# 21cmfast/21cmFAST

Hardware: AMD Instinct MI355X
Metric: IonizeBox cells/sec (512^3 HII_DIM, 40 filter radii) (higher is better)
Workload: dtype f32; 1 GPU; ComputeIonizedBox single-z, HII_DIM=512, 40 filter steps, G=2 (delta tophat + n_ion exp-MFP), first snapshot, device-resident inputs; hii_dim=512, n_radii=40, filtered_grids=2, parallelism=single GPU, fft=native

## Files before the change

### 21cmfast_amd/csrc/hip/c21hip.h

```cpp
#ifndef C21HIP_H
#define C21HIP_H

#include <stddef.h>

#include "ws_slots.h"

#ifdef __cplusplus
extern "C" {
#endif

int c21hip_device_count(void);
int c21hip_current_device(void);
int c21hip_use_device(int device);
int c21hip_is_device_ptr(const void *p);
void *c21hip_ws(int slot, size_t bytes);
__attribute__((visibility("hidden"))) const void *c21_stage_in(int slot, const void *p, size_t bytes, void *stream, int *status);
void *c21hip_ws_peek(int slot, size_t *bytes);
int c21hip_ws_adopt(int slot, void *ptr, size_t bytes);
void *c21hip_raw_alloc(size_t bytes);
void *c21hip_vmm_chunk(size_t phys_bytes, size_t map_bytes, void **va_out);
void c21hip_vmm_chunk_free(void *chunk);
int c21hip_ws_adopt_vmm(int slot, void *chunk, size_t bytes);
void c21hip_raw_free(void *p);
size_t c21hip_free_bytes(void);
// ... 37 lines not shown
                           void *stream);
int c21hip_split_filter_c2r(const float *split_src, float *split_work, float *real_out,
                            long out_zstride, int nx, int ny, int nz, double box_len,
                            double box_len_z, int filter_type, float R, float R_param, int apply,
                            void *stream);

int c21hip_split_r2c(const float *real_in, long in_zstride, float *split_out, int nx, int ny,
                     int nz, double factor, double lo, double hi, float out_scale, void *stream);
int c21hip_split_filter_xy(const float *split_src, float *split_work, int nx, int ny, int nz,
                           double box_len, double box_len_z, int filter_type, float R,
                           float R_param, int apply, void *stream);
int c21hip_split_filter_xy2(const float *src_a, float *work_a, int filter_a, float R_param_a,
                            const float *src_b, float *work_b, int filter_b, float R_param_b,
                            int nx, int ny, int nz, double box_len, double box_len_z, float R,
                            int apply, int table_slot, int tables_ready, void *stream);
int c21hip_split_filter_shell(const float *src_a, float *work_a, int filter_a, const float *src_b,
                              float *work_b, int filter_b, int n_grids, int nx, int ny, int nz,
                              double box_len, double box_len_z, float R_inner, float R_outer,
                              float R_star, int apply, void *stream);
int c21hip_split_filter_xy2_pair(const float *src_a, float *work_a, float *work_a2, int filter_a,
                                 float R_param_a, const float *src_b, float *work_b,
                                 float *work_b2, int filter_b, float R_param_b, int nx, int ny,
                                 int nz, double box_len, double box_len_z, float R, float R2,
                                 int table_slot, int table_slot2, int phases, void *stream);
int c21hip_split_filter_x_pair1(const float *src, float *work, float *work2, int filter_type, int nx, int ny,
                                int nz, double box_len, double box_len_z, float R, float R2, int phases,
                                void *stream);
int c21hip_split_filter_xy2_pair_eval(const float *src_a, float *work_a, float *work_a2, int filter_a,
                                      const float *src_b, float *work_b, float *work_b2, int filter_b, int nx,
                                      int ny, int nz, double box_len, double box_len_z, float R, float R2,
// ... 591 lines not shown
```

### 21cmfast_amd/csrc/hip/fft_native.hip

```cpp
#include <hip/hip_runtime.h>

#include <cmath>
#include <map>
#include <mutex>
#include <vector>

#include "c21hip.h"
#include "fcoll_device.h"
#include "ms_window.h"
#include "c21cm_abi.h"
#include "c21cm_grid.h"

#ifndef C21X_XPAIR_THREADS
#define C21X_XPAIR_THREADS 512
#endif
#ifndef C21X_FUSE512
#define C21X_FUSE512 1
#endif
#ifndef C21X_FUSE1024
#define C21X_FUSE1024 1
#endif
#ifndef C21X_F512_MERGE
#define C21X_F512_MERGE 1
#endif
// ... 505 lines not shown
    long line_stride, line_bstride, outer_stride, outer_bstride, col_stride;
    int line_lb, outer_lb;
    int n_outer, filter_axis;
    int og, ct, npair;
    const wtab_t *wt0, *wt1;
};

template <int N, int SIGN, int FMODE>
__global__ void __launch_bounds__((LineThreads<N, FMODE>::value), (LineThreads<N, FMODE>::value / 256))
line_pass_kernel(LinePassArgs a, const float2 *__restrict__ tw_global) {
    static_assert(N >= 64, "tile loader needs N >= 64");
    constexpr int kBlock = LineThreads<N, FMODE>::value;
    constexpr int TZ = line_tile_cols(N);
    constexpr int CPAIR = TZ / 2;
    constexpr int RSTEP = kBlock / CPAIR;
    constexpr bool WEVAL = (FMODE >= 6 && FMODE <= 9);
    constexpr bool WDIRECT = (FMODE == 8 || FMODE == 9);
    constexpr bool WIN = (FMODE == 3 || (FMODE == 5 && !C21X_XPAIR_NOWIN) || WEVAL);
    constexpr bool PAIR = (FMODE == 5 || FMODE == 7 || FMODE == 9);
    constexpr int NR = PAIR ? 2 : 1;
    using LineItem = LineItemT<PAIR>;
    extern __shared__ float4 lds_raw[];
    float2 *tile = reinterpret_cast<float2 *>(lds_raw);
    float2 *tw = tile + NR * N * TZ;
    float2 *tw_half = tw + N;
    float *wnodes = reinterpret_cast<float *>(tw_half + (N >= 1024 ? N / 2 : 0));
    for (int t = threadIdx.x; t < N; t += kBlock) tw[t] = tw_global[t];
    if (N >= 1024)
        for (int t = threadIdx.x; t < N / 2; t += kBlock) tw_half[t] = tw_global[2 * t];
    if constexpr (WEVAL) {
        const int per = 3 * a.wev_n_nodes;
        for (int t = threadIdx.x; t < per; t += kBlock) {
// ... 98 lines not shown
        const int outer = mi == 0 ? it.og : it.n_outer - it.og;
        return (long)(outer >> it.outer_lb) * it.outer_bstride +
               (long)(outer & ((1 << it.outer_lb) - 1)) * it.outer_stride +
               (long)it.ct * TZ * it.col_stride;
    };
    auto row_off = [](const LineItem &it, int r) {
        return (unsigned)(r >> it.line_lb) * (unsigned)it.line_bstride +
               (unsigned)(r & ((1 << it.line_lb) - 1)) * (unsigned)it.line_stride;
    };

    constexpr bool TWO_SETS = (N < 1024) && (!PAIR || C21X_XPAIR_TWO_SETS);
    float4 reg_a[2 * NP], reg_b[2 * NP];
    constexpr bool F512 = C21X_FUSE512 && N == 512 && kBlock == 512 && (FMODE == 0 || WEVAL);
    constexpr bool F1024 = C21X_FUSE1024 && N == 1024 && kBlock == 512 && (FMODE == 0 || FMODE == 3 || WEVAL);
    constexpr bool FUSED = F512 || F1024;
    constexpr int NW = FUSED ? 2 * NP : NP;
    constexpr bool WPRE = (N >= 512) && !FUSED;
    float2 wpre[NR][WPRE ? NP : 1], wcur[NR][NW], wpre_half[NR], wcur_half[NR];
    auto w_reload = [&](const LineItem &it, int m) {
        const int mi = it.npair == 2 ? (m & 1) : 0;
        return m == 0 || (a.dual && mi == 0);
    };
    struct KAbs {
        float kh, kl;
    };
    auto k_abs = [](float kx, float ky, float kz) -> KAbs {
        const float ksq = __fadd_rn(__fadd_rn(__fmul_rn(kx, kx), __fmul_rn(ky, ky)), __fmul_rn(kz, kz));
        KAbs k;
        k.kh = __builtin_amdgcn_sqrtf(ksq);
        const float r = __fmaf_rn(-k.kh, k.kh, ksq);
// ... 215 lines not shown
    auto process = [&](float4(&reg)[2 * NP], const TileRef &cur, const TileRef &nxt,
                       const TileRef &refill) {
        const LineItem &it = cur.it;
        const int m = cur.m;
        const long st_half = (long)((N / 2) >> it.line_lb) * it.line_bstride;
        if (!first) __syncthreads();
        first = false;
        if (WIN && WPRE && w_reload(it, m)) {
#pragma unroll
            for (int rr = 0; rr < NR; rr++) {
#pragma unroll
                for (int u = 0; u < NP; u++) wcur[rr][u] = wpre[rr][WPRE ? u : 0];
                wcur_half[rr] = wpre_half[rr];
            }
        }
        double op_c0 = 1., op_c1 = 1.;
        if (FMODE == 4) {
            const int c0 = it.ct * TZ + 2 * c4;
            int kyi0, kyi1, kzi0, kzi1;
            if (it.filter_axis == 0) {
                const int mi = it.npair == 2 ? (m & 1) : 0;
                const int outer = mi == 0 ? it.og : it.n_outer - it.og;
                kyi0 = kyi1 = (outer <= a.n_y / 2) ? outer : outer - a.n_y;
                kzi0 = c0;
                kzi1 = c0 + 1;
            } else {
                kyi0 = (c0 <= a.n_y / 2) ? c0 : c0 - a.n_y;
                kyi1 = (c0 + 1 <= a.n_y / 2) ? c0 + 1 : c0 + 1 - a.n_y;
                kzi0 = kzi1 = a.n_z / 2;
            }
// ... 883 lines not shown
    hipStream_t stream;
    KTimeScope(int kind, hipStream_t s) : stream(s) {
        if (!g_ktime_on) return;
        if (hipEventCreate(&r.e0) != hipSuccess || hipEventCreate(&r.e1) != hipSuccess) return;
        r.kind = kind;
        (void)hipEventRecord(r.e0, stream);
    }
    ~KTimeScope() {
        if (r.kind < 0) return;
        (void)hipEventRecord(r.e1, stream);
        g_ktime.push_back(r);
    }
};
constexpr int ktime_kind(int sign, int fmode) {
    return sign < 0 ? 9 : (fmode == 0 ? 1 : fmode == 3 ? 0 : fmode == 5 ? 6 : (fmode == 6 || fmode == 8) ? 7
                                                              : (fmode == 7 || fmode == 9) ? 8 : 10);
}

static bool ynyq_split_on() {
    static int on = -1;
    if (on < 0) {
        const char *e = getenv("C21CM_YNYQ_SPLIT");
        on = (e && atoi(e) == 0) ? 0 : 1;
    }
    return on != 0;
}

#ifndef C21X_XORDER_DEFAULT
#define C21X_XORDER_DEFAULT 3
#endif
template <int N, int SIGN, int FMODE>
int launch_line_pass_mode(const LinePassArgs &a, hipStream_t stream) {
    const float2 *tw = twiddles(N);
    if (!tw) {
        c21hip_set_error("native FFT: twiddle table allocation failed");
        return C21CM_MEMORY_ALLOC_ERROR;
    }
    const size_t lds = sizeof(float2) * ((size_t)((FMODE == 5 || FMODE == 7 || FMODE == 9) ? 2 : 1) * N *
                                             line_tile_cols(N) + N + (N >= 1024 ? N / 2 : 0)) +
                       ((FMODE >= 6 && FMODE <= 9) ? sizeof(float) * 3 * (size_t)a.wev_n_nodes * a.wev_n_tabs : 0);
    if (lds > 160 * 1024) {
        c21hip_set_error("native FFT: %zu bytes of LDS for a %d-point line pass (mode %d)", lds, N, FMODE);
        return C21CM_VALUE_ERROR;
    }
    if (FMODE != 0 && a.n_geo > 1 && a.g1_strided) {
        c21hip_set_error("native FFT: a strided second geometry in a line pass of mode %d", FMODE);
        return C21CM_VALUE_ERROR;
    }
    const bool epi_split = ynyq_split_on() && a.n_geo > 1 && a.g1_strided && a.g1.line_bstride == 1 &&
                           a.g1.line_lb == 0 && a.g1.col_stride % 2 == 0;
    const int n_work = geo_items(a.g0) + (a.n_geo > 1 ? geo_items(a.g1) : 0);
    int per_cu = (int)((160 * 1024) / lds) > 0 ? (int)((160 * 1024) / lds) : 1;
    const int by_waves = (LineThreads<N, FMODE>::value >= 512 && N > 256) ? 1 : 2;
    if (per_cu > by_waves) per_cu = by_waves;
    int nblocks = 256 * per_cu;
// ... 23 lines not shown
}

template <int N, int SIGN>
int launch_line_pass(const LinePassArgs &a, int fmode, hipStream_t stream) {
    if (SIGN > 0 && fmode == 3) return launch_line_pass_mode<N, +1, 3>(a, stream);
    if (SIGN > 0 && fmode == 4) return launch_line_pass_mode<N, +1, 4>(a, stream);
    if constexpr (N <= 512)
        if (SIGN > 0 && fmode == 5) return launch_line_pass_mode<N, +1, 5>(a, stream);
    if constexpr (N >= 128 && (N & (N - 1)) == 0) {
        if (SIGN > 0 && fmode == 6) return launch_line_pass_mode<N, +1, 6>(a, stream);
        if (SIGN > 0 && fmode == 8) return launch_line_pass_mode<N, +1, 8>(a, stream);
        if constexpr (N <= 512) {
            if (SIGN > 0 && fmode == 7) return launch_line_pass_mode<N, +1, 7>(a, stream);
            if (SIGN > 0 && fmode == 9) return launch_line_pass_mode<N, +1, 9>(a, stream);
        }
    }
    if (fmode >= 6 && fmode <= 9) {
        c21hip_set_error("native FFT: evaluated windows are not built for %d-point lines", N);
        return C21CM_VALUE_ERROR;
    }
    return launch_line_pass_mode<N, SIGN, 0>(a, stream);
}

template <int SIGN>
int dispatch_line_pass(int n, const LinePassArgs &a, int fmode, hipStream_t stream) {
    switch (n) {
        case 64: return launch_line_pass<64, SIGN>(a, fmode, stream);
        case 128: return launch_line_pass<128, SIGN>(a, fmode, stream);
        case 192: return launch_line_pass<192, SIGN>(a, fmode, stream);
        case 256: return launch_line_pass<256, SIGN>(a, fmode, stream);
// ... 1828 lines not shown
    if (env && env[0] == 't') return 0;
    return wev_static_ok(filter_a, filter_b, n_grids, nx, ny, nz, 1, nullptr, nullptr) ? 1 : 0;
}
extern "C" int c21hip_split_filter_xy_single_pair(const float *src, float *work, float *work2,
                                                  int filter_type, float R_param, int nx, int ny,
                                                  int nz, double box_len, double box_len_z, float R,
                                                  float R2, int phases, void *stream_) {
    if (!g_wev.active) {
        c21hip_set_error("single-grid pair sweep: needs a prepared window set (c21hip_wev_prepare)");
        return C21CM_VALUE_ERROR;
    }
    return filter_xy_pair(src, work, work2, filter_type, R_param, nullptr, nullptr, nullptr, 0, 0.f,
                          nx, ny, nz, box_len, box_len_z, R, R2, 0, 1, phases & ~1, stream_, 1);
}

extern "C" int c21hip_split_r2c(const float *real_in, long in_zstride, float *split_out, int nx,
                                int ny, int nz, double factor, double lo, double hi,
                                float out_scale, void *stream_) {
    hipStream_t stream = (hipStream_t)stream_;
    if (!c21hip_native_fft_supported(nx, ny, nz)) {
        c21hip_set_error("native FFT does not support %dx%dx%d", nx, ny, nz);
        return C21CM_VALUE_ERROR;
    }
    const int H = nz / 2;
    const long nlines = (long)nx * ny;
    float2 *o_main = reinterpret_cast<float2 *>(split_out);
    float2 *o_nyq = o_main + nlines * H;
    ZFwdArgs z{};
    z.ny = ny;
    z.lb = split_xb_log2(nx);
    z.in = real_in;
    z.in_zstride = in_zstride;
    z.main = o_main;
// ... 4 lines not shown
    int st = dispatch_z_r2c(nz, z, nlines, stream);
    if (st) return st;
    LinePassArgs a{};
    a.fp.type = -1;
    a.n_y = ny;
    a.n_z = nz;
    a.out_scale = 1.0f;
    a.n_geo = 2;
    a.n_grids = 1;
    a.g0 = geo_y_main(nx, ny, H, line_tile_cols(ny), split_xb_log2(nx));
    a.g1 = geo_y_nyq(nx, ny, line_tile_cols(ny));
    a.g1_strided = 1;
    geo_ptrs(a.g0, 0, o_main, o_main);
    geo_ptrs(a.g1, 0, o_nyq, o_nyq);
    if ((st = dispatch_line_pass<-1>(ny, a, 0, stream))) return st;
    a.out_scale = out_scale;
    a.g0 = geo_x_main(ny, H, line_tile_cols(nx), split_xb_log2(nx));
    a.g1 = geo_x_nyq(ny, line_tile_cols(nx));
    a.g1_strided = 0;
    geo_ptrs(a.g0, 0, o_main, o_main);
    geo_ptrs(a.g1, 0, o_nyq, o_nyq);
    return dispatch_line_pass<-1>(nx, a, 0, stream);
}

extern "C" int c21hip_split_z_c2r(const float *split_work, float *real_out, long out_zstride,
                                  int nx, int ny, int nz, void *stream) {
    const long nlines = (long)nx * ny;
    ZPassArgs z{};
    z.ny = ny;
    z.lb = split_xb_log2(nx);
    z.main = reinterpret_cast<const float2 *>(split_work);
    z.nyq = z.main + nlines * (nz / 2);
    z.out = real_out;
    z.out_zstride = out_zstride;
    z.out_scale = 1.0f;
    return dispatch_z_c2r(nz, z, nlines, (hipStream_t)stream);
}
// ... 832 lines not shown
```

### 21cmfast_amd/csrc/host/ionize_driver.c

```c
#include <math.h>
#include <stdio.h>
#include <stdlib.h>
#include <string.h>

#include "../hip/c21hip.h"
#include "c21cm_grid.h"

#define MAX_COPYBACK 12
typedef struct {
    void *host[MAX_COPYBACK];
    void *dev[MAX_COPYBACK];
    size_t bytes[MAX_COPYBACK];
    int n;
} copyback_list;

#define SC_SUMS 0
#define SC_MEANS (SC_SUMS + C21CM_MAX_RADII)
#define SC_MINMAX (SC_MEANS + C21CM_MAX_RADII)
#define SC_XHSUM (SC_MINMAX + 4)
#define SC_FLAG (SC_XHSUM + 1)
#define SC_G12SUM (SC_FLAG + 1)
#define SC_SUMS_M (SC_G12SUM + 1)
#define SC_MEANS_M (SC_SUMS_M + C21CM_MAX_RADII)
#define SC_MINMAX_M (SC_MEANS_M + C21CM_MAX_RADII)
// ... 172 lines not shown
    const float *whalo_sfr, *prev_nrec;
    float *G12, *mfp, *nrec_out;
    double *rr_dev;
    int pair_radii;
    const float *density, *n_ion, *xe_dense, *Tneutral, *prev_zre;
    float *xH, *zre, *Tk, *nion_dense;
    double *scalars;
    double *partials;
    float *table_dev;
    int fused;
    double *def_partials;
    long def_stride;
    int def_first, def_step, def_count;
    int tab_seq;
    int wev;
    int fused_rc;
    int eul_pend, eul_pend_buf;
    unsigned char *eul_pend_mask;
    float *nion_dense2;
    int band_off;
    int band_used;
    int band_next;
    int band_pend;
    int band_h1, band_h2, band_hn;
    unsigned char *band_mask;
    const unsigned char *r0_mask;
    int r0_slab, r0_cb, r0_ce;
    int band_mf;
    int band_skip;
    short band_hist[C21CM_MAX_RADII][3];
// ... 11 lines not shown
    float *eul_xe[2];
    int wev_pair, pairx_R;
    float *pairx_buf;
    int sphere;
    int mini, lag_mini;
    float *pd_unf, *pd_work, *pd_fil, *mta_unf, *mta_work, *mta_fil, *mtm_unf, *mtm_work, *mtm_fil;
    const float *prev_density, *mta_dense, *mtm_dense, *hist_a, *hist_m;
    float *mini_tables, *nion_all, *mini_all;
    int eul_mask;
    copyback_list cb;
    size_t cb_cell0, cb_ncell;
} ion_ctx;

static int r0_direct(void);

static int g_loop_flags;
int c21cm_ionize_last_loop_flags(void) { return g_loop_flags; }

static int ctx_setup(ion_ctx *c, const c21cm_ionize_spec *s, const PerturbedField *pf,
                     const IonizedBox *prev, const TsBox *ts, const HaloBox *halos,
                     IonizedBox *box, int need_outputs, int fused_rc_ok, void *stream) {
    int status = 0;
    memset(c, 0, sizeof(*c));
    c->s = s;
    c->stream = stream;
    c->nx = s->hii_dim;
    c->ny = s->hii_dim;
    c->nz = s->hii_dim_z;
    c->ntot = (size_t)c->nx * c->ny * c->nz;
    c->npad = (size_t)c->nx * c->ny * 2 * (size_t)(c->nz / 2 + 1);
// ... 267 lines not shown
    g_spectra.stars_r0_ready = 0;
    g_spectra.nx = c->nx;
    g_spectra.nz = c->nz;
    g_spectra.ts = c->s->use_ts_fluct;
    g_spectra.density = pf->density;
    g_spectra.n_ion = c->lagrangian ? halos->n_ion : NULL;
    g_spectra.xe = c->s->use_ts_fluct ? ts->xray_ionised_fraction : NULL;
    g_spectra.factor = c->s->photoncons_adjustment_factor;
}

static int prepare_grid(ion_ctx *c, const float *dense, float *cgrid, float *scratch,
                        double factor, double lo, double hi) {
    int status = 0;
    (void)scratch;
    if (c->native) {
        TRY(c21hip_split_r2c(dense, c->nz, cgrid, c->nx, c->ny, c->nz, factor, lo, hi,
                             1.0f / (float)c->ntot, c->stream));
        goto done;
    }
    float *padded = cgrid;
    TRY(c21hip_pack_clip(dense, padded, c->nx, c->ny, c->nz, factor, lo, hi, c->stream));
    TRY(c21hip_fft_r2c(padded, c->nx, c->ny, c->nz, c->stream));
    TRY(c21hip_divide_inplace(padded, c->npad, (float)c->ntot, c->stream));
done:
    return status;
}

static int filter_to_real(ion_ctx *c, const float *unf, float *work, float *fil, int filter_type,
                          float R, float R_param, int apply) {
    int status = 0;
    const c21cm_ionize_spec *s = c->s;
    if (c->native) {
        TRY(c21hip_split_filter_c2r(unf, work, fil, 2 * (long)(c->nz / 2 + 1), c->nx, c->ny, c->nz,
                                    s->box_len, s->box_len_z, filter_type, R, R_param, apply,
                                    c->stream));
    } else {
        TRY(c21hip_copy_filter(unf, fil, c->nx, c->ny, c->nz, s->box_len, s->box_len_z,
                               filter_type, R, R_param, apply, c->stream));
        TRY(c21hip_fft_c2r(fil, c->nx, c->ny, c->nz, c->stream));
    }
done:
    return status;
}

static int preloop(ion_ctx *c) {
    int status = 0;
    const c21cm_ionize_spec *s = c->s;
    TRY(prepare_grid(c, c->density, c->delta_unf, c->delta_fil, s->photoncons_adjustment_factor,
                     -1., 1e6));
    if (c->lagrangian) TRY(prepare_grid(c, c->n_ion, c->stars_unf, c->stars_fil, 1., 0., 1e20));
    if (s->use_ts_fluct) TRY(prepare_grid(c, c->xe_dense, c->xe_unf, c->xe_fil, 1., 0., 1.));
    if (c->recomb && c->lagrangian)
        TRY(prepare_grid(c, c->whalo_sfr, c->sfr_unf, c->sfr_fil, 1., 0., 1e20));
    if (c->filter_rec) TRY(prepare_grid(c, c->prev_nrec, c->nrec_unf, c->nrec_fil, 1., 0., 1e20));
    if (c->mini) {
        TRY(prepare_grid(c, c->prev_density, c->pd_unf, c->pd_fil, 1., -1., 1e6));
        TRY(prepare_grid(c, c->mtm_dense, c->mtm_unf, c->mtm_fil, 1., -INFINITY, INFINITY));
// ... 157 lines not shown
    const int set = c->tab_seq & 1;
    const int buf_a = 2 * set, buf_b = 2 * set + 1;
    tab_init();
    const int tab_async = !c->wev && g_tab.enabled && c->ntot >= ((size_t)1 << 26);
    if (tab_async) {
        if (c->tab_seq == 0) {
            TRY(c21hip_event_record(g_tab.ev_sync, c->stream));
            TRY(c21hip_stream_wait_event(g_tab.aux, g_tab.ev_sync));
            TRY(tab_build_async(c, R_a, buf_a));
            if (R_b >= 1) TRY(tab_build_async(c, R_b, buf_b));
        }
        if (next_a >= 1) TRY(tab_build_async(c, next_a, 2 * (set ^ 1)));
        if (next_b >= 1) TRY(tab_build_async(c, next_b, 2 * (set ^ 1) + 1));
        TRY(c21hip_stream_wait_event(c->stream, g_tab.ev_table[buf_a]));
        if (R_b >= 1) TRY(c21hip_stream_wait_event(c->stream, g_tab.ev_table[buf_b]));
    }
    if (R_b >= 1) {
        static int yy = -1;
        if (yy < 0) {
            const char *e = getenv("C21CM_PAIR_ORDER");
            yy = (e && e[0] == 'y') ? 1 : 0;
        }
        const float *xw[2] = {c->fused_rc ? c->sfr_work : (s->use_ts_fluct ? c->xe_work : NULL),
                              c->fused_rc ? c->sfr_work2 : (s->use_ts_fluct ? c->xe_work2 : NULL)};
        const float *xe_of[2] = {c->x3_on ? c->x3_work : NULL, c->x3_on ? c->x3_work2 : NULL};
        for (int ph = 0; ph < 3; ph++) {
            const int bits = ph == 0 ? (tab_async ? 2 : 3) : (4 << (ph - 1));
            TRY(c21hip_split_filter_xy2_pair(
                c->delta_unf, c->delta_work, c->delta_work2, s->hii_filter, 0.f, c->stars_unf,
                c->stars_work, c->stars_work2, s->stars_filter, (float)s->mfp_meandens, c->nx,
// ... 36 lines not shown
                c->cur_x4 = c->x4_work;
                TRY(z_ionise_radius(c, R_a, c->delta_work, c->stars_work, xw[0], first_cross));
            }
        }
        c->tab_seq++;
        if (yy) {
            c->cur_xe = xe_of[0];
            c->cur_x4 = c->x4_work;
            TRY(z_ionise_radius(c, R_a, c->delta_work, c->stars_work, xw[0], first_cross));
        }
        c->cur_xe = xe_of[1];
        c->cur_x4 = c->x4_work2;
        TRY(z_ionise_radius(c, R_b, c->delta_work2, c->stars_work2, xw[1], first_cross));
        goto done;
    } else {
        TRY(c21hip_split_filter_xy2(c->delta_unf, c->delta_work, s->hii_filter, 0.f, c->stars_unf,
                                    c->stars_work, s->stars_filter, (float)s->mfp_meandens, c->nx,
                                    c->ny, c->nz, s->box_len, s->box_len_z, (float)s->R[R_a], 1,
                                    buf_a, tab_async, c->stream));
        if (c->x3_on)
            TRY(c21hip_split_filter_xy_shared(c->x3_unf, c->x3_work, s->hii_filter, c->nx, c->ny,
                                              c->nz, s->box_len, s->box_len_z, (float)s->R[R_a], 1,
                                              buf_a, c->stream));
        if (c->fused_rc)
            TRY(c21hip_split_filter_xy(c->sfr_unf, c->sfr_work, c->nx, c->ny, c->nz, s->box_len,
                                       s->box_len_z, s->stars_filter, (float)s->R[R_a],
                                       (float)s->mfp_meandens, 1, c->stream));
        if (c->x4_on)
            TRY(c21hip_split_filter_xy_shared(c->x4_unf, c->x4_work, s->hii_filter, c->nx, c->ny,
                                              c->nz, s->box_len, s->box_len_z, (float)s->R[R_a], 1,
// ... 29 lines not shown
            status = C21CM_VALUE_ERROR;
            goto done;
        }
        c->rec0 = 0.;
        if (!c->inhomo) {
            float r0 = 0.f;
            if (c21hip_is_device_ptr(c->prev_nrec)) {
                TRY(c21hip_d2h(&r0, c->prev_nrec, sizeof(float), c->stream));
                TRY(c21hip_sync(c->stream));
            } else {
                r0 = c->prev_nrec[0];
            }
            c->rec0 = (double)r0;
        }
    }
    int R_a = first;
    while (R_a >= lowest) {
        const int want_b = c->pair_radii && R_a - step >= lowest;
        const int R_b = want_b ? R_a - step : -1;
        const int n_a = (want_b ? R_b : R_a) - step;
        const int next_a = n_a >= lowest ? n_a : -1;
        const int next_b = (c->pair_radii && next_a >= 1 && next_a - step >= lowest) ? next_a - step
                                                                                     : -1;
        TRY(fused_step(c, R_a, R_b, first_cross, next_a, next_b));
        R_a = n_a;
    }
done:
    c21hip_wev_release();
    c->wev = 0;
    return status;
}

static int eul_xe_buffers(ion_ctx *c) {
    if (c->eul_xe[0] && c->eul_xe[1]) return 0;
    c->eul_xe[0] = (float *)c21hip_ws(WS_EUL_XE0, c->ntot * sizeof(float));
    c->eul_xe[1] = (float *)c21hip_ws(WS_EUL_XE1, c->ntot * sizeof(float));
    return (c->eul_xe[0] && c->eul_xe[1]) ? 0 : C21CM_MEMORY_ALLOC_ERROR;
}

static int mini_radius(ion_ctx *c, int R_ct, const c21hip_ionize_args *args, int apply, float R) {
    int status = 0;
    const c21cm_ionize_spec *s = c->s;
// ... 1028 lines not shown
}

int c21cm_ionize_grids(const c21cm_ionize_spec *spec, const PerturbedField *perturbed_field,
                       const IonizedBox *previous_ionize_box, const TsBox *spin_temp,
                       const HaloBox *halos, IonizedBox *box, c21cm_ionize_report *report,
                       void *stream) {
    int status = validate_spec(spec, perturbed_field, halos, spin_temp, box);
    if (status) return status;
    ion_ctx c;
    phase_clock clk = {{NULL}, 0, 0};
    unsigned char *mask = NULL;
    g_spectra.valid = 0;
    TRY(ctx_setup(&c, spec, perturbed_field, previous_ionize_box, spin_temp, halos, box, 1, 1, stream));
    TRY(clock_start(&clk, 4, stream));
    TRY(init_output_grids(&c, previous_ionize_box));
    TRY(preloop(&c));
    TRY(clock_mark(&clk, stream));
    if (c.fused || c.eul_mask || c.sphere) {
        mask = (unsigned char *)c21hip_ws(WS_FIRST_CROSS, c.ntot);
        if (!mask) {
            status = C21CM_MEMORY_ALLOC_ERROR;
            goto done;
        }
        cross_bits_begin(&c);
        if (!c.cross_bits)
            TRY(c21hip_memset(mask, 0, c.ntot, stream));
    }
    TRY(native_wev_prepare(&c));
    if (mask) {
        TRY(radii_ladder(&c, spec->n_radii - 1, 1, mask, spec->r_lowest == 0 ? 0 : -1));
// ... 58 lines not shown
static int radii_phase_box(const c21cm_ionize_spec *spec, const PerturbedField *pf, const HaloBox *halos,
                           const TsBox *ts, int recomb, IonizedBox *dummy) {
    memset(dummy, 0, sizeof(*dummy));
    if (spec && spec->fcoll_mode != C21CM_FCOLL_STARS_GRID)
        dummy->unnormalised_nion = (float *)c21hip_ws(
            WS_NION_DENSE, (size_t)spec->hii_dim * spec->hii_dim * spec->hii_dim_z * sizeof(float));
    IonizedBox probe = *dummy;
    float sentinel;
    probe.neutral_fraction = probe.z_reion = probe.kinetic_temperature = &sentinel;
    if (recomb) probe.ionisation_rate_G12 = probe.cumulative_recombinations = &sentinel;
    int status = validate_spec(spec, pf, halos, ts, &probe);
    if (!status && spec->use_mini_halos) status = no_mini_shards();
    return status;
}

static int radii_phase_preloop(ion_ctx *c, const PerturbedField *pf, const HaloBox *halos, const TsBox *ts) {
    g_spectra.valid = 0;
    const int status = preloop(c);
    if (!status) spectra_remember(c, pf, halos, ts);
    return status;
}

static int spectra_reuse(ion_ctx *c, const PerturbedField *pf, const HaloBox *halos, const TsBox *ts,
                         int *stars_ready) {
    int status = 0;
    if (spectra_match(c, pf, halos, ts)) {
        if (stars_ready) *stars_ready = g_spectra.stars_r0_ready;
    } else {
        status = preloop(c);
    }
    g_spectra.valid = 0;
    return status;
// ... 34 lines not shown
                             const HaloBox *halos, unsigned char *first_cross,
                             c21cm_ionize_report *report, void *stream) {
    IonizedBox dummy;
    int status = 0;
    if (!first_cross || !c21hip_is_device_ptr(first_cross) || world < 1 || rank < 0 ||
        rank >= world) {
        c21hip_set_error("ionize shard: first_cross must be a device array, 0 <= rank < world");
        return C21CM_VALUE_ERROR;
    }
    if ((status = radii_phase_box(spec, perturbed_field, halos, spin_temp, 0, &dummy))) return status;
    ion_ctx c;
    phase_clock clk = {{NULL}, 0, 0};
    TRY(ctx_setup(&c, spec, perturbed_field, previous_ionize_box, spin_temp, halos, &dummy, 0, 0, stream));
    TRY(clock_start(&clk, 3, stream));
    TRY(c21hip_memset(first_cross, 0, c.ntot, stream));
    TRY(radii_phase_preloop(&c, perturbed_field, halos, spin_temp));
    TRY(clock_mark(&clk, stream));
    TRY(native_wev_prepare(&c));
    TRY(radii_ladder(&c, spec->n_radii - 1 - rank, world, first_cross, -1));
    TRY(flush_deferred(&c));
    if (c.fused && spec->r_lowest == 0 && rank == (spec->n_radii - 1) % world && !r0_direct()) {
        TRY(final_prepare(&c));
        g_spectra.stars_r0_ready = 1;
    }
    TRY(clock_mark(&clk, stream));
    TRY(radii_phase_report(&c, world, &clk, report));
done:
    c21hip_wev_release();
    clock_free(&clk);
    return status;
}

int c21cm_ionize_shard_finish(const c21cm_ionize_spec *spec, const unsigned char *first_cross,
                              const PerturbedField *perturbed_field,
                              const IonizedBox *previous_ionize_box, const TsBox *spin_temp,
                              const HaloBox *halos, IonizedBox *box, c21cm_ionize_report *report,
                              void *stream) {
    int status = validate_spec(spec, perturbed_field, halos, spin_temp, box);
    if (!status && spec->use_mini_halos) status = no_mini_shards();
    if (status) return status;
    if (!first_cross || !c21hip_is_device_ptr(first_cross)) {
        c21hip_set_error("ionize shard: first_cross must be a device array");
// ... 158 lines not shown
    phase_clock clk = {{NULL}, 0, 0};
    TRY(ctx_setup(&c, spec, perturbed_field, previous_ionize_box, spin_temp, halos, &dummy, 0, 0, stream));
    const size_t ntot = c.ntot;
    c.xH = (float *)c21hip_ws(WS_SH_XH, ntot * sizeof(float));
    c.zre = (float *)c21hip_ws(WS_SH_ZRE, ntot * sizeof(float));
    c.G12 = (float *)c21hip_ws(WS_SH_G12, ntot * sizeof(float));
    c.mfp = (float *)c21hip_ws(WS_SH_MFP, ntot * sizeof(float));
    if (!c.xH || !c.zre || !c.G12 || !c.mfp) {
        status = C21CM_MEMORY_ALLOC_ERROR;
        goto done;
    }
    TRY(clock_start(&clk, 3, stream));
    TRY(c21hip_fill(c.xH, ntot, 1.0f, stream));
    TRY(c21hip_memset(c.G12, 0, ntot * sizeof(float), stream));
    TRY(c21hip_memset(c.mfp, 0, ntot * sizeof(float), stream));
    TRY(radii_phase_preloop(&c, perturbed_field, halos, spin_temp));
    TRY(clock_mark(&clk, stream));
    TRY(native_wev_prepare(&c));
    for (int R_ct = spec->n_radii - 1 - rank; R_ct >= 1 && R_ct >= spec->r_lowest; R_ct -= world)
        TRY(one_radius(&c, R_ct, NULL, -1));
    TRY(c21hip_pack_cross_keys(c.mfp, c.G12, cross_keys, ntot, stream));
    TRY(clock_mark(&clk, stream));
    TRY(radii_phase_report(&c, world, &clk, report));
done:
    c21hip_wev_release();
    clock_free(&clk);
    return status;
}

int c21cm_ionize_shard_finish_keys(const c21cm_ionize_spec *spec,
                                   const unsigned long long *cross_keys,
// ... 68 lines not shown
        return C21CM_VALUE_ERROR;
    }
    if ((status = radii_phase_box(spec, perturbed_field, halos, spin_temp, 1, &dummy))) return status;
    ion_ctx c;
    phase_clock clk = {{NULL}, 0, 0};
    TRY(ctx_setup(&c, spec, perturbed_field, previous_ionize_box, spin_temp, halos, &dummy, 0, 1, stream));
    if (!c.fused_rc) {
        c21hip_set_error("ionize shard: the fused recombination loop is not available for this box");
        status = C21CM_VALUE_ERROR;
        goto done;
    }
    c.G12 = cross_g12;
    TRY(clock_start(&clk, 3, stream));
    TRY(c21hip_memset(first_cross, 0, c.ntot, stream));
    TRY(c21hip_memset(cross_g12, 0, c.ntot * sizeof(float), stream));
    TRY(radii_phase_preloop(&c, perturbed_field, halos, spin_temp));
    TRY(clock_mark(&clk, stream));
    TRY(radii_ladder(&c, spec->n_radii - 1 - rank, world, first_cross, -1));
    TRY(flush_deferred(&c));
    TRY(clock_mark(&clk, stream));
    TRY(radii_phase_report(&c, world, &clk, report));
done:
    c21hip_wev_release();
    clock_free(&clk);
    return status;
}

int c21cm_ionize_shard_finish_rc(const c21cm_ionize_spec *spec, const unsigned char *first_cross,
                                 const float *cross_g12, const PerturbedField *perturbed_field,
                                 const IonizedBox *previous_ionize_box, const TsBox *spin_temp,
                                 const HaloBox *halos, IonizedBox *box,
                                 c21cm_ionize_report *report, void *stream) {
    int status = validate_spec(spec, perturbed_field, halos, spin_temp, box);
    if (status) return status;
    if (!first_cross || !cross_g12 || !c21hip_is_device_ptr(first_cross) ||
        !c21hip_is_device_ptr(cross_g12) || !c21cm_ionize_shard_rc_supported(spec)) {
        c21hip_set_error("ionize shard: first_cross / cross_g12 must be device arrays of a spec that "
// ... 117 lines not shown
```

Measured before the change: 3.503 billion cells/s.

## Fuse forward X-pass FFT into first radius filter/inverse X sweep

Defers the forward X-axis FFT of the delta and stars spectra during preloop (doing only z and y passes), then runs it inside a new line-pass mode that does forward X, stores the spectrum, applies the evaluated window, and runs the inverse X in one kernel for the first radius. The point is to save one full read/write sweep of both spectra. To get a single-radius opening sweep, the ladder is changed so that with an odd count of paired radii the first radius runs alone. That changes how radii are paired and adds a larger kernel with extra syncs.

```diff
diff --git a/21cmfast_amd/csrc/hip/c21hip.h b/21cmfast_amd/csrc/hip/c21hip.h
--- a/21cmfast_amd/csrc/hip/c21hip.h
+++ b/21cmfast_amd/csrc/hip/c21hip.h
@@ -75,6 +75,13 @@
                             const float *src_b, float *work_b, int filter_b, float R_param_b,
                             int nx, int ny, int nz, double box_len, double box_len_z, float R,
                             int apply, int table_slot, int tables_ready, void *stream);
+int c21hip_split_fwdx_filter_xy2(float *spec_a, float *work_a, int filter_a, float R_param_a, float *spec_b,
+                                 float *work_b, int filter_b, float R_param_b, int nx, int ny, int nz,
+                                 double box_len, double box_len_z, float R, float out_scale, int phases,
+                                 void *stream);
+int c21hip_fwdx_fused_supported(int nx, int ny, int nz);
+int c21hip_split_r2c_zy(const float *real_in, long in_zstride, float *split_out, int nx, int ny, int nz,
+                        double factor, double lo, double hi, void *stream);
 int c21hip_split_filter_shell(const float *src_a, float *work_a, int filter_a, const float *src_b,
                               float *work_b, int filter_b, int n_grids, int nx, int ny, int nz,
                               double box_len, double box_len_z, float R_inner, float R_outer,
diff --git a/21cmfast_amd/csrc/hip/fft_native.hip b/21cmfast_amd/csrc/hip/fft_native.hip
--- a/21cmfast_amd/csrc/hip/fft_native.hip
+++ b/21cmfast_amd/csrc/hip/fft_native.hip
@@ -543,8 +543,9 @@
     constexpr int TZ = line_tile_cols(N);
     constexpr int CPAIR = TZ / 2;
     constexpr int RSTEP = kBlock / CPAIR;
-    constexpr bool WEVAL = (FMODE >= 6 && FMODE <= 9);
-    constexpr bool WDIRECT = (FMODE == 8 || FMODE == 9);
+    constexpr bool WEVAL = (FMODE >= 6 && FMODE <= 11);
+    constexpr bool WDIRECT = (FMODE == 8 || FMODE == 9 || FMODE == 11);
+    constexpr bool FWDX = (FMODE == 10 || FMODE == 11);
     constexpr bool WIN = (FMODE == 3 || (FMODE == 5 && !C21X_XPAIR_NOWIN) || WEVAL);
     constexpr bool PAIR = (FMODE == 5 || FMODE == 7 || FMODE == 9);
     constexpr int NR = PAIR ? 2 : 1;
@@ -673,6 +674,7 @@
     constexpr bool F512 = C21X_FUSE512 && N == 512 && kBlock == 512 && (FMODE == 0 || WEVAL);
     constexpr bool F1024 = C21X_FUSE1024 && N == 1024 && kBlock == 512 && (FMODE == 0 || FMODE == 3 || WEVAL);
     constexpr bool FUSED = F512 || F1024;
+    static_assert(!FWDX || F512, "the forward + inverse sweep is built for 512-point lines on the F512 path");
     constexpr int NW = FUSED ? 2 * NP : NP;
     constexpr bool WPRE = (N >= 512) && !FUSED;
     float2 wpre[NR][WPRE ? NP : 1], wcur[NR][NW], wpre_half[NR], wcur_half[NR];
@@ -918,6 +920,131 @@
                 wcur_half[rr] = wpre_half[rr];
             }
         }
+        if constexpr (FWDX) {
+            auto twf = [](float2 w, auto sg) __attribute__((always_inline)) {
+                return decltype(sg)::value == SIGN ? w : make_float2(w.x, -w.y);
+            };
+            const int obase = (r0 & 7) + 64 * (r0 >> 3);
+            auto stage1 = [&](float2(&c0)[8], float2(&c1)[8], auto sg) __attribute__((always_inline)) {
+                constexpr int SG = decltype(sg)::value;
+                Dft<8, SG>::run(c0);
+                Dft<8, SG>::run(c1);
+#pragma unroll
+                for (int j = 0; j < 8; j++) {
+                    float2 o0 = c0[j], o1 = c1[j];
+                    if (j > 0) {
+                        const float2 w = twf(twd1[F512_ ? j : 0], sg);
+                        o0 = cmul(o0, w);
+                        o1 = cmul(o1, w);
+                    }
+                    *reinterpret_cast<float4 *>(tile + (8 * r0 + j) * TZ + 2 * c4) =
+                        make_float4(o0.x, o0.y, o1.x, o1.y);
+                }
+            };
+            auto stage2 = [&](auto sg) __attribute__((always_inline)) {
+                constexpr int SG = decltype(sg)::value;
+                float2 s0[8], s1[8];
+#pragma unroll
+                for (int k = 0; k < 8; k++) {
+                    const float4 t = *reinterpret_cast<const float4 *>(tile + (r0 + RSTEP * k) * TZ + 2 * c4);
+                    s0[k] = make_float2(t.x, t.y);
+                    s1[k] = make_float2(t.z, t.w);
+                }
+                __syncthreads();
+                float2 w2[8];
+                if (!C21X_F512_HOIST2) {
+                    const int ps = r0 & ~7;
+                    w2[1] = tw[ps];
+                    w2[2] = tw[2 * ps];
+                    w2[4] = tw[4 * ps];
+                    w2[3] = cmul(w2[1], w2[2]);
+                    w2[5] = cmul(w2[1], w2[4]);
+                    w2[6] = cmul(w2[2], w2[4]);
+                    w2[7] = cmul(w2[3], w2[4]);
+                    if (SG > 0)
+#pragma unroll
+                        for (int j = 1; j < 8; j++) w2[j].y = -w2[j].y;
+                }
+                Dft<8, SG>::run(s0);
+                Dft<8, SG>::run(s1);
+#pragma unroll
+                for (int j = 0; j < 8; j++) {
+                    float2 o0 = s0[j], o1 = s1[j];
+                    if (j > 0) {
+                        const float2 w = C21X_F512_HOIST2 ? twf(twd2[F512_ ? j : 0], sg) : w2[j];
+                        o0 = cmul(o0, w);
+                        o1 = cmul(o1, w);
+                    }
+                    *reinterpret_cast<float4 *>(tile + (obase + 8 * j) * TZ + 2 * c4) =
+                        make_float4(o0.x, o0.y, o1.x, o1.y);
+                }
+                __syncthreads();
+            };
+            auto stage3 = [&](float2(&c0)[8], float2(&c1)[8], auto sg) __attribute__((always_inline)) {
+                constexpr int SG = decltype(sg)::value;
+#pragma unroll
+                for (int k = 0; k < 8; k++) {
+                    const float4 t = *reinterpret_cast<const float4 *>(tile + (r0 + RSTEP * k) * TZ + 2 * c4);
+                    c0[k] = make_float2(t.x, t.y);
+                    c1[k] = make_float2(t.z, t.w);
+                }
+                Dft<8, SG>::run(c0);
+                Dft<8, SG>::run(c1);
+            };
+            auto store_rows = [&](float2 *st, const float4(&v)[8]) __attribute__((always_inline)) {
+#pragma unroll
+                for (int j = 0; j < 8; j++) {
+                    const int row = r0 + RSTEP * j;
+                    const unsigned roff = row_off(it, row < N / 2 ? row : row - N / 2);
+                    float2 *p = st + (row < N / 2 ? 0 : st_half);
+                    *reinterpret_cast<float4 *>(p + (roff + 2u * c4)) = v[j];
+                }
+            };
+            const std::integral_constant<int, -1> fwd{};
+            const std::integral_constant<int, +1> inv{};
+            float2 c0[8], c1[8];
+            float4 v[8];
+#pragma unroll
+            for (int u = 0; u < 8; u++) {
+                c0[u] = make_float2(reg[u].x, reg[u].y);
+                c1[u] = make_float2(reg[u].z, reg[u].w);
+            }
+            stage1(c0, c1, fwd);
+            __syncthreads();
+            issue_loads(reg, refill.it, refill.m);
+            stage2(fwd);
+            stage3(c0, c1, fwd);
+#pragma unroll
+            for (int j = 0; j < 8; j++) {
+                v[j] = make_float4(c0[j].x, c0[j].y, c1[j].x, c1[j].y);
+                if (a.out_scale != 1.0f) {
+                    v[j].x *= a.out_scale;
+                    v[j].y *= a.out_scale;
+                    v[j].z *= a.out_scale;
+                    v[j].w *= a.out_scale;
+                }
+            }
+            store_rows((member_grid(it, m) ? it.dst1 : it.dst0) + member_base(it, m), v);
+#pragma unroll
+            for (int u = 0; u < 8; u++) {
+                const float2 wv = wcur[0][u];
+                c0[u] = make_float2(__fmul_rn(v[u].x, wv.x), __fmul_rn(v[u].y, wv.x));
+                c1[u] = make_float2(__fmul_rn(v[u].z, wv.y), __fmul_rn(v[u].w, wv.y));
+            }
+            __syncthreads();
+            stage1(c0, c1, inv);
+            __syncthreads();
+            stage2(inv);
+            stage3(c0, c1, inv);
+#pragma unroll
+            for (int j = 0; j < 8; j++) v[j] = make_float4(c0[j].x, c0[j].y, c1[j].x, c1[j].y);
+            const bool nyq = cur.work >= n_work0;
+            store_rows((member_grid(it, m) ? (nyq ? a.g1.dst2[1] : a.g0.dst2[1]) : (nyq ? a.g1.dst2[0] : a.g0.dst2[0])) +
+                           member_base(it, m),
+                       v);
+            if (w_reload(nxt.it, nxt.m)) issue_wloads(nxt.it, nxt.m);
+            return;
+        }
         double op_c0 = 1., op_c1 = 1.;
         if (FMODE == 4) {
             const int c0 = it.ct * TZ + 2 * c4;
@@ -1831,7 +1958,8 @@
 };
 constexpr int ktime_kind(int sign, int fmode) {
     return sign < 0 ? 9 : (fmode == 0 ? 1 : fmode == 3 ? 0 : fmode == 5 ? 6 : (fmode == 6 || fmode == 8) ? 7
-                                                              : (fmode == 7 || fmode == 9) ? 8 : 10);
+                                                              : (fmode == 7 || fmode == 9) ? 8
+                                                              : (fmode == 10 || fmode == 11) ? 11 : 10);
 }
 
 static bool ynyq_split_on() {
@@ -1855,7 +1983,7 @@
     }
     const size_t lds = sizeof(float2) * ((size_t)((FMODE == 5 || FMODE == 7 || FMODE == 9) ? 2 : 1) * N *
                                              line_tile_cols(N) + N + (N >= 1024 ? N / 2 : 0)) +
-                       ((FMODE >= 6 && FMODE <= 9) ? sizeof(float) * 3 * (size_t)a.wev_n_nodes * a.wev_n_tabs : 0);
+                       ((FMODE >= 6 && FMODE <= 11) ? sizeof(float) * 3 * (size_t)a.wev_n_nodes * a.wev_n_tabs : 0);
     if (lds > 160 * 1024) {
         c21hip_set_error("native FFT: %zu bytes of LDS for a %d-point line pass (mode %d)", lds, N, FMODE);
         return C21CM_VALUE_ERROR;
@@ -1909,6 +2037,14 @@
             if (SIGN > 0 && fmode == 7) return launch_line_pass_mode<N, +1, 7>(a, stream);
             if (SIGN > 0 && fmode == 9) return launch_line_pass_mode<N, +1, 9>(a, stream);
         }
+    }
+    if constexpr (N == 512 && C21X_FUSE512) {
+        if (SIGN > 0 && fmode == 10) return launch_line_pass_mode<N, +1, 10>(a, stream);
+        if (SIGN > 0 && fmode == 11) return launch_line_pass_mode<N, +1, 11>(a, stream);
+    }
+    if (fmode >= 10) {
+        c21hip_set_error("native FFT: the forward pass X is fused into the sweep of 512-point lines only, not %d", N);
+        return C21CM_VALUE_ERROR;
     }
     if (fmode >= 6 && fmode <= 9) {
         c21hip_set_error("native FFT: evaluated windows are not built for %d-point lines", N);
@@ -3767,9 +3903,8 @@
                           nx, ny, nz, box_len, box_len_z, R, R2, 0, 1, phases & ~1, stream_, 1);
 }
 
-extern "C" int c21hip_split_r2c(const float *real_in, long in_zstride, float *split_out, int nx,
-                                int ny, int nz, double factor, double lo, double hi,
-                                float out_scale, void *stream_) {
+static int split_r2c(const float *real_in, long in_zstride, float *split_out, int nx, int ny, int nz,
+                     double factor, double lo, double hi, float out_scale, bool pass_x, void *stream_) {
     hipStream_t stream = (hipStream_t)stream_;
     if (!c21hip_native_fft_supported(nx, ny, nz)) {
         c21hip_set_error("native FFT does not support %dx%dx%d", nx, ny, nz);
@@ -3804,6 +3939,7 @@
     geo_ptrs(a.g0, 0, o_main, o_main);
     geo_ptrs(a.g1, 0, o_nyq, o_nyq);
     if ((st = dispatch_line_pass<-1>(ny, a, 0, stream))) return st;
+    if (!pass_x) return 0;
     a.out_scale = out_scale;
     a.g0 = geo_x_main(ny, H, line_tile_cols(nx), split_xb_log2(nx));
     a.g1 = geo_x_nyq(ny, line_tile_cols(nx));
@@ -3811,6 +3947,72 @@
     geo_ptrs(a.g0, 0, o_main, o_main);
     geo_ptrs(a.g1, 0, o_nyq, o_nyq);
     return dispatch_line_pass<-1>(nx, a, 0, stream);
+}
+
+extern "C" int c21hip_split_r2c(const float *real_in, long in_zstride, float *split_out, int nx,
+                                int ny, int nz, double factor, double lo, double hi,
+                                float out_scale, void *stream_) {
+    return split_r2c(real_in, in_zstride, split_out, nx, ny, nz, factor, lo, hi, out_scale, true, stream_);
+}
+
+extern "C" int c21hip_split_r2c_zy(const float *real_in, long in_zstride, float *split_out, int nx,
+                                   int ny, int nz, double factor, double lo, double hi, void *stream_) {
+    return split_r2c(real_in, in_zstride, split_out, nx, ny, nz, factor, lo, hi, 1.0f, false, stream_);
+}
+
+extern "C" int c21hip_fwdx_fused_supported(int nx, int ny, int nz) {
+    return (C21X_FUSE512 && nx == 512 && c21hip_native_fft_supported(nx, ny, nz)) ? 1 : 0;
+}
+
+extern "C" int c21hip_split_fwdx_filter_xy2(float *spec_a, float *work_a, int filter_a, float R_param_a,
+                                            float *spec_b, float *work_b, int filter_b, float R_param_b,
+                                            int nx, int ny, int nz, double box_len, double box_len_z,
+                                            float R, float out_scale, int phases, void *stream_) {
+    const int ft[2] = {filter_a, filter_b};
+    const float rp[2] = {R_param_a, R_param_b};
+    int st = check_filter_request(2, nx, ny, nz, ft, 1);
+    if (st) return st;
+    if (!c21hip_fwdx_fused_supported(nx, ny, nz)) {
+        c21hip_set_error("fused forward pass X: not built for %dx%dx%d (512-point x-lines only)", nx, ny, nz);
+        return C21CM_VALUE_ERROR;
+    }
+    hipStream_t stream = (hipStream_t)stream_;
+    const int H = nz / 2;
+    const long nlines = (long)nx * ny;
+    LinePassArgs a{};
+    a.fp.type = -1;
+    a.n_y = ny;
+    a.n_z = nz;
+    a.n_geo = 2;
+    a.n_grids = 2;
+    float2 *spec[2] = {reinterpret_cast<float2 *>(spec_a), reinterpret_cast<float2 *>(spec_b)};
+    float2 *work[2] = {reinterpret_cast<float2 *>(work_a), reinterpret_cast<float2 *>(work_b)};
+    if (phases & 2) {
+        if (!wev_use(a, 2, ft, rp, R, R, false, nx, ny, nz, box_len, box_len_z)) {
+            c21hip_set_error("fused forward pass X: no prepared window set holds radius %g", (double)R);
+            return C21CM_VALUE_ERROR;
+        }
+        a.out_scale = out_scale;
+        a.g0 = geo_x_main(ny, H, line_tile_cols(nx), split_xb_log2(nx));
+        a.g1 = geo_x_nyq(ny, line_tile_cols(nx));
+        for (int g = 0; g < 2; g++) {
+            geo_ptrs(a.g0, g, spec[g], spec[g]);
+            geo_ptrs(a.g1, g, spec[g] + nlines * H, spec[g] + nlines * H);
+            a.g0.dst2[g] = work[g];
+            a.g1.dst2[g] = work[g] + nlines * H;
+        }
+        if ((st = dispatch_line_pass<+1>(nx, a, g_wev.covers ? 10 : 11, stream))) return st;
+    }
+    if (!(phases & 4)) return 0;
+    a.out_scale = 1.0f;
+    a.g0 = geo_y_main(nx, ny, H, line_tile_cols(ny), split_xb_log2(nx));
+    a.g1 = geo_y_nyq(nx, ny, line_tile_cols(ny));
+    a.g1_strided = 1;
+    for (int g = 0; g < 2; g++) {
+        geo_ptrs(a.g0, g, work[g], work[g]);
+        geo_ptrs(a.g1, g, work[g] + nlines * H, work[g] + nlines * H);
+    }
+    return dispatch_line_pass<+1>(ny, a, 0, stream);
 }
 
 extern "C" int c21hip_split_z_c2r(const float *split_work, float *real_out, long out_zstride,
diff --git a/21cmfast_amd/csrc/host/ionize_driver.c b/21cmfast_amd/csrc/host/ionize_driver.c
--- a/21cmfast_amd/csrc/host/ionize_driver.c
+++ b/21cmfast_amd/csrc/host/ionize_driver.c
@@ -210,6 +210,7 @@
     int def_first, def_step, def_count;
     int tab_seq;
     int wev;
+    int fwdx_defer;
     int fused_rc;
     int eul_pend, eul_pend_buf;
     unsigned char *eul_pend_mask;
@@ -251,6 +252,24 @@
 
 static int r0_direct(void);
 
+static int ladder_head(void) {
+    static int head = -1;
+    if (head < 0) {
+        const char *e = getenv("C21CM_LADDER");
+        head = (e && e[0] == 't') ? 0 : 1;
+    }
+    return head;
+}
+
+static int fwdx_fuse_on(void) {
+    static int on = -1;
+    if (on < 0) {
+        const char *e = getenv("C21CM_FWDX_FUSE");
+        on = (e && e[0] == '0') ? 0 : 1;
+    }
+    return on;
+}
+
 static int g_loop_flags;
 int c21cm_ionize_last_loop_flags(void) { return g_loop_flags; }
 
@@ -548,6 +567,10 @@
     int status = 0;
     (void)scratch;
     if (c->native) {
+        if (c->fwdx_defer && (cgrid == c->delta_unf || cgrid == c->stars_unf)) {
+            TRY(c21hip_split_r2c_zy(dense, c->nz, cgrid, c->nx, c->ny, c->nz, factor, lo, hi, c->stream));
+            goto done;
+        }
         TRY(c21hip_split_r2c(dense, c->nz, cgrid, c->nx, c->ny, c->nz, factor, lo, hi,
                              1.0f / (float)c->ntot, c->stream));
         goto done;
@@ -575,6 +598,23 @@
     }
 done:
     return status;
+}
+
+static int ladder_count(int first, int step, int lowest) {
+    if (lowest < 1) lowest = 1;
+    return first < lowest ? 0 : (first - lowest) / step + 1;
+}
+
+static int ladder_lone_first(const ion_ctx *c, int n) {
+    return n >= 1 && (!c->pair_radii || n == 1 || ((n & 1) && ladder_head()));
+}
+
+static void fwdx_plan(ion_ctx *c, int first, int step) {
+    const c21cm_ionize_spec *s = c->s;
+    c->fwdx_defer = c->fused && c->lagrangian && fwdx_fuse_on() &&
+                    c21hip_fwdx_fused_supported(c->nx, c->ny, c->nz) &&
+                    c21hip_wev_applicable(s->hii_filter, s->stars_filter, 2, c->nx, c->ny, c->nz) &&
+                    ladder_lone_first(c, ladder_count(first, step, s->r_lowest));
 }
 
 static int preloop(ion_ctx *c) {
@@ -762,6 +802,12 @@
         if (next_b >= 1) TRY(tab_build_async(c, next_b, 2 * (set ^ 1) + 1));
         TRY(c21hip_stream_wait_event(c->stream, g_tab.ev_table[buf_a]));
         if (R_b >= 1) TRY(c21hip_stream_wait_event(c->stream, g_tab.ev_table[buf_b]));
+    }
+    if (c->fwdx_defer && (R_b >= 1 || !c->wev)) {
+        c21hip_set_error("ionize: the forward pass X was left to a single-radius sweep with evaluated windows, "
+                         "and the ladder opens with none");
+        status = C21CM_VALUE_ERROR;
+        goto done;
     }
     if (R_b >= 1) {
         static int yy = -1;
@@ -828,6 +874,14 @@
         TRY(z_ionise_radius(c, R_b, c->delta_work2, c->stars_work2, xw[1], first_cross));
         goto done;
     } else {
+        if (c->fwdx_defer) {
+            TRY(c21hip_split_fwdx_filter_xy2(c->delta_unf, c->delta_work, s->hii_filter, 0.f, c->stars_unf,
+                                             c->stars_work, s->stars_filter, (float)s->mfp_meandens, c->nx,
+                                             c->ny, c->nz, s->box_len, s->box_len_z, (float)s->R[R_a],
+                                             1.0f / (float)c->ntot, 6, c->stream));
+            c->fwdx_defer = 0;
+            g_loop_flags |= 128;
+        } else
         TRY(c21hip_split_filter_xy2(c->delta_unf, c->delta_work, s->hii_filter, 0.f, c->stars_unf,
                                     c->stars_work, s->stars_filter, (float)s->mfp_meandens, c->nx,
                                     c->ny, c->nz, s->box_len, s->box_len_z, (float)s->R[R_a], 1,
@@ -887,9 +941,12 @@
             c->rec0 = (double)r0;
         }
     }
+    const int n_radii = ladder_count(first, step, lowest);
+    const int lone_first = n_radii > 1 && ladder_lone_first(c, n_radii);
+    if (c->pair_radii && n_radii > 1 && (n_radii & 1)) g_loop_flags |= lone_first ? 64 : 256;
     int R_a = first;
     while (R_a >= lowest) {
-        const int want_b = c->pair_radii && R_a - step >= lowest;
+        const int want_b = c->pair_radii && !(lone_first && R_a == first) && R_a - step >= lowest;
         const int R_b = want_b ? R_a - step : -1;
         const int n_a = (want_b ? R_b : R_a) - step;
         const int next_a = n_a >= lowest ? n_a : -1;
@@ -899,6 +956,10 @@
         R_a = n_a;
     }
 done:
+    if (!status && c->fwdx_defer) {
+        c21hip_set_error("ionize: the fused loop ended with the forward pass X of its spectra still owed");
+        status = C21CM_VALUE_ERROR;
+    }
     c21hip_wev_release();
     c->wev = 0;
     return status;
@@ -1957,6 +2018,7 @@
     TRY(ctx_setup(&c, spec, perturbed_field, previous_ionize_box, spin_temp, halos, box, 1, 1, stream));
     TRY(clock_start(&clk, 4, stream));
     TRY(init_output_grids(&c, previous_ionize_box));
+    fwdx_plan(&c, spec->n_radii - 1, 1);
     TRY(preloop(&c));
     TRY(clock_mark(&clk, stream));
     if (c.fused || c.eul_mask || c.sphere) {
@@ -2045,8 +2107,10 @@
     return status;
 }
 
-static int radii_phase_preloop(ion_ctx *c, const PerturbedField *pf, const HaloBox *halos, const TsBox *ts) {
+static int radii_phase_preloop(ion_ctx *c, const PerturbedField *pf, const HaloBox *halos, const TsBox *ts,
+                               int first, int step) {
     g_spectra.valid = 0;
+    fwdx_plan(c, first, step);
     const int status = preloop(c);
     if (!status) spectra_remember(c, pf, halos, ts);
     return status;
@@ -2111,7 +2175,7 @@
     TRY(ctx_setup(&c, spec, perturbed_field, previous_ionize_box, spin_temp, halos, &dummy, 0, 0, stream));
     TRY(clock_start(&clk, 3, stream));
     TRY(c21hip_memset(first_cross, 0, c.ntot, stream));
-    TRY(radii_phase_preloop(&c, perturbed_field, halos, spin_temp));
+    TRY(radii_phase_preloop(&c, perturbed_field, halos, spin_temp, spec->n_radii - 1 - rank, world));
     TRY(clock_mark(&clk, stream));
     TRY(native_wev_prepare(&c));
     TRY(radii_ladder(&c, spec->n_radii - 1 - rank, world, first_cross, -1));
@@ -2123,6 +2187,7 @@
     TRY(clock_mark(&clk, stream));
     TRY(radii_phase_report(&c, world, &clk, report));
 done:
+    if (status) g_spectra.valid = 0;
     c21hip_wev_release();
     clock_free(&clk);
     return status;
@@ -2311,7 +2376,7 @@
     TRY(c21hip_fill(c.xH, ntot, 1.0f, stream));
     TRY(c21hip_memset(c.G12, 0, ntot * sizeof(float), stream));
     TRY(c21hip_memset(c.mfp, 0, ntot * sizeof(float), stream));
-    TRY(radii_phase_preloop(&c, perturbed_field, halos, spin_temp));
+    TRY(radii_phase_preloop(&c, perturbed_field, halos, spin_temp, -1, 1));
     TRY(clock_mark(&clk, stream));
     TRY(native_wev_prepare(&c));
     for (int R_ct = spec->n_radii - 1 - rank; R_ct >= 1 && R_ct >= spec->r_lowest; R_ct -= world)
@@ -2410,13 +2475,14 @@
     TRY(clock_start(&clk, 3, stream));
     TRY(c21hip_memset(first_cross, 0, c.ntot, stream));
     TRY(c21hip_memset(cross_g12, 0, c.ntot * sizeof(float), stream));
-    TRY(radii_phase_preloop(&c, perturbed_field, halos, spin_temp));
+    TRY(radii_phase_preloop(&c, perturbed_field, halos, spin_temp, spec->n_radii - 1 - rank, world));
     TRY(clock_mark(&clk, stream));
     TRY(radii_ladder(&c, spec->n_radii - 1 - rank, world, first_cross, -1));
     TRY(flush_deferred(&c));
     TRY(clock_mark(&clk, stream));
     TRY(radii_phase_report(&c, world, &clk, report));
 done:
+    if (status) g_spectra.valid = 0;
     c21hip_wev_release();
     clock_free(&clk);
     return status;
```

Result: no change. 3.513 billion cells/s, median of 6 (+0.3%).
